# forgi86/pyMPC

Measured on AMD Instinct MI355X. Metric: QP-solves/sec (MPC steps/sec) at nx=12 nu=4 Np=30; max |u*-u*_ref|, higher is better.
Workload: dtype f64

## Files before the change

### pympc_amd/csrc/mpcqp_latw.h

```cpp
#pragma once

constexpr int latw_owner(int , int , int kind, int t) { return kind == 1 ? NWAVES - 1 - t % NWAVES : t % NWAVES; }
constexpr bool latw_fused(int N) { return (N + 3) / 4 == NWAVES; }
constexpr int LATW_F0 = 6;
constexpr int LATW_FB = 6;
constexpr int latw_slot(int N, int W, int Lq, int kq, int tq) {
    int s = latw_fused(N) ? LATW_F0 : 0;
    for (int pass = 0; pass < 2; ++pass)
        for (int li = 0; li < 2; ++li) {
            const int L = pass == 0 ? li : 1 - li;
            for (int kind = (pass == 0 ? 0 : 2); kind < (pass == 0 ? 2 : 3); ++kind)
                for (int t = 0; t < lat_count(N, L, kind); ++t) {
                    if (latw_fused(N) && L == 0 && kind < 2) continue;
                    if (latw_fused(N) && kind == 2) continue;
                    if (L == Lq && kind == kq && t == tq) return s;
                    if (latw_owner(N, L, kind, t) == W) s += lat_nfr(N, L, kind, t);
                }
        }
    return s;
}
constexpr int latw_back_base(int N, int W) { return latw_slot(N, W, -1, -1, -1); }
constexpr int latw_slots(int N, int W) { return latw_slot(N, W, -1, -1, -1) + (latw_fused(N) ? LATW_FB : 0); }
constexpr int latw_max_slots(int N) { int m = 0; for (int w = 0; w < NWAVES; ++w) m = latw_slots(N, w) > m ? latw_slots(N, w) : m; return m; }
constexpr int latw_top_stage(int r) { return 4 * (r + 1) - 1; }

#define LATW_TOP_LDS(N) ((BcrFmt::top_count(N) * BcrFmt::top_count(N) + 2) * BcrFmt::NN + 32 * BcrFmt::top_count(N))
#if NT == 512
#define LATW_DISPATCH(wv, CALL) switch (wv) { \
    case 0: { constexpr int W = 0; CALL; } break; case 1: { constexpr int W = 1; CALL; } break; \
    case 2: { constexpr int W = 2; CALL; } break; case 3: { constexpr int W = 3; CALL; } break; \
    case 4: { constexpr int W = 4; CALL; } break; case 5: { constexpr int W = 5; CALL; } break; \
    case 6: { constexpr int W = 6; CALL; } break; default: { constexpr int W = 7; CALL; } break; }
#else
#define LATW_DISPATCH(wv, CALL) LAT_DISPATCH(wv, CALL)
#endif

template <int N, int W>
__device__ __forceinline__ void latw_load(const double *F, d4 *fr) {
    const int lane = threadIdx.x & 63;
    if constexpr (latw_fused(N)) {
        constexpr int s0 = 4 * W;
        if constexpr (s0 < N) { fr[0] = bcr_frag(F, s0, BcrFmt::ODINV, lane); fr[2] = bcr_frag(F, s0, BcrFmt::OLBRT, lane); }
        if constexpr (s0 + 2 < N) { fr[1] = bcr_frag(F, s0 + 2, BcrFmt::ODINV, lane); fr[3] = bcr_frag(F, s0 + 2, BcrFmt::OLBLT, lane); }
        if constexpr (s0 + 3 < N) fr[4] = bcr_frag(F, s0 + 2, BcrFmt::OLBRT, lane);
        if constexpr (W > 0 && s0 < N) fr[5] = bcr_frag(F, s0, BcrFmt::OLBLT, lane);
    }
    if constexpr (latw_fused(N)) {
        constexpr int bb = latw_back_base(N, W), e1 = 4 * W + 1, ea = 4 * W, eb = 4 * W + 2;
        if constexpr (e1 < N) { if constexpr (e1 - 2 >= 0) fr[bb] = bcr_frag(F, e1, BcrFmt::OLBL, lane); if constexpr (e1 + 2 < N) fr[bb + 1] = bcr_frag(F, e1, BcrFmt::OLBR, lane); }
        if constexpr (ea < N) { if constexpr (ea - 1 >= 0) fr[bb + 2] = bcr_frag(F, ea, BcrFmt::OLBL, lane); if constexpr (ea + 1 < N) fr[bb + 3] = bcr_frag(F, ea, BcrFmt::OLBR, lane); }
        if constexpr (eb < N) { fr[bb + 4] = bcr_frag(F, eb, BcrFmt::OLBL, lane); if constexpr (eb + 1 < N) fr[bb + 5] = bcr_frag(F, eb, BcrFmt::OLBR, lane); }
    }
    static_for<0, 2>([&](auto lc) {
        constexpr int L = decltype(lc)::value, h = 1 << L;
        static_for<0, lat_count(N, L, 0)>([&](auto tc) {
            constexpr int t = decltype(tc)::value, i = lat_stage(L, 0, t);
            if constexpr (!(latw_fused(N) && L == 0) && latw_owner(N, L, 0, t) == W) {
                constexpr int s = latw_slot(N, W, L, 0, t);
                fr[s] = bcr_frag(F, i - h, BcrFmt::OLBRT, lane);
                if constexpr (i + h < N) fr[s + 1] = bcr_frag(F, i + h, BcrFmt::OLBLT, lane);
            }
        });
        static_for<0, lat_count(N, L, 1)>([&](auto tc) {
            constexpr int t = decltype(tc)::value, e = lat_stage(L, 1, t);
            if constexpr (!(latw_fused(N) && L == 0) && latw_owner(N, L, 1, t) == W) { constexpr int s1 = latw_slot(N, W, L, 1, t); fr[s1] = bcr_frag(F, e, BcrFmt::ODINV, lane); }
            if constexpr (!latw_fused(N) && latw_owner(N, L, 2, t) == W) {
                constexpr int s = latw_slot(N, W, L, 2, t);
                if constexpr (e - h >= 0) fr[s] = bcr_frag(F, e, BcrFmt::OLBL, lane);
                constexpr int s2 = s + (e - h >= 0 ? 1 : 0);
                if constexpr (e + h < N) fr[s2] = bcr_frag(F, e, BcrFmt::OLBR, lane);
            }
        });
    });
}

struct LatwVecs { double *tb, *cb; const double *t1, *t2, *t3, *c1, *c2, *c3; double *xt, *x2; };
template <bool FROMC>
__device__ __forceinline__ void latw_mv_lds(const d4 a, const LatwVecs &v, int off, double &p, double &q) {
    const double i0 = FROMC ? v.cb[off] : v.tb[off], i1 = FROMC ? v.c1[off] : v.t1[off], i2 = FROMC ? v.c2[off] : v.t2[off], i3 = FROMC ? v.c3[off] : v.t3[off];
    p = __builtin_amdgcn_mfma_f64_4x4x4f64(a[0], i0, p, 0, 0, 0);
    q = __builtin_amdgcn_mfma_f64_4x4x4f64(a[2], i2, q, 0, 0, 0);
    p = __builtin_amdgcn_mfma_f64_4x4x4f64(a[1], i1, p, 0, 0, 0);
    q = __builtin_amdgcn_mfma_f64_4x4x4f64(a[3], i3, q, 0, 0, 0);
}

template <int N, int W, int L>
__device__ __forceinline__ void latw_fwd(const d4 *fr, const LatwVecs &v) {
    constexpr int h = 1 << L;
    static_for<0, lat_count(N, L, 0)>([&](auto tc) {
        constexpr int t = decltype(tc)::value, i = lat_stage(L, 0, t);
        if constexpr (latw_owner(N, L, 0, t) == W) {
            constexpr int s = latw_slot(N, W, L, 0, t);
            double p = v.tb[i * 16], q = 0.0;
            if constexpr (latw_fused(N) && L == 1) p += v.x2[((i + 1) / 4 - 1) * 16];
            latw_mv_lds<false>(fr[s], v, (i - h) * 16, p, q);
            if constexpr (i + h < N) latw_mv_lds<false>(fr[s + 1], v, (i + h) * 16, p, q);
            if constexpr (L == 1) v.xt[((i + 1) / 4 - 1) * 16] = p + q;
            else v.tb[i * 16] = p + q;
        }
    });
    static_for<0, lat_count(N, L, 1)>([&](auto tc) {
        constexpr int t = decltype(tc)::value, e = lat_stage(L, 1, t);
        if constexpr (latw_owner(N, L, 1, t) == W) {
            constexpr int s1 = latw_slot(N, W, L, 1, t);
            double p = 0.0, q = 0.0;
            latw_mv_lds<false>(fr[s1], v, e * 16, p, q);
            v.cb[e * 16] = p + q;
        }
    });
}
template <int N, int W>
__device__ __forceinline__ void latw_fwd0_own(const d4 *fr, const LatwVecs &v) {
    constexpr int s0 = 4 * W;
    if constexpr (s0 < N) { double p = 0.0, q = 0.0; latw_mv_lds<false>(fr[0], v, s0 * 16, p, q); v.cb[s0 * 16] = p + q; }
    if constexpr (s0 + 2 < N) { double p = 0.0, q = 0.0; latw_mv_lds<false>(fr[1], v, (s0 + 2) * 16, p, q); v.cb[(s0 + 2) * 16] = p + q; }
    if constexpr (s0 + 1 < N) {
        double p = v.tb[(s0 + 1) * 16], q = 0.0;
        latw_mv_lds<false>(fr[2], v, s0 * 16, p, q);
        if constexpr (s0 + 2 < N) latw_mv_lds<false>(fr[3], v, (s0 + 2) * 16, p, q);
        v.tb[(s0 + 1) * 16] = p + q;
    }
    if constexpr (s0 + 3 < N) { double p = v.tb[(s0 + 3) * 16], q = 0.0; latw_mv_lds<false>(fr[4], v, (s0 + 2) * 16, p, q); v.tb[(s0 + 3) * 16] = p + q; }
    if constexpr (W > 0 && s0 < N) { double p = 0.0, q = 0.0; latw_mv_lds<false>(fr[5], v, s0 * 16, p, q); v.x2[(W - 1) * 16] = p + q; }
}
template <int N, int W, int L, bool TOPIN>
__device__ __forceinline__ void latw_bwd(const d4 *fr, const LatwVecs &v) {
    constexpr int h = 1 << L;
    static_for<0, lat_count(N, L, 2)>([&](auto tc) {
        constexpr int t = decltype(tc)::value, e = lat_stage(L, 2, t);
        if constexpr (latw_owner(N, L, 2, t) == W) {
            constexpr int s = latw_slot(N, W, L, 2, t), s2 = s + (e - h >= 0 ? 1 : 0);
            double p = v.cb[e * 16], q = 0.0;
            if constexpr (e - h >= 0) latw_mv_lds<TOPIN>(fr[s], v, (e - h) * 16, p, q);
            if constexpr (e + h < N) latw_mv_lds<TOPIN>(fr[s2], v, (e + h) * 16, p, q);
            v.tb[e * 16] = p + q;
        }
    });
}

template <int N, int W>
__device__ __forceinline__ void latw_bwd1(const d4 *fr, const LatwVecs &v) {
    static_for<0, BcrFmt::top_count(N)>([&](auto rc) {
        constexpr int r = decltype(rc)::value;
        if constexpr (r % NWAVES == W) v.tb[latw_top_stage(r) * 16] = v.cb[latw_top_stage(r) * 16];
    });
    latw_bwd<N, W, 1, true>(fr, v);
}

template <int N, int W>
__device__ __forceinline__ void latw_bwd_own(const d4 *fr, const LatwVecs &v) {
    constexpr int bb = latw_back_base(N, W), e1 = 4 * W + 1, ea = 4 * W, eb = 4 * W + 2;
    if constexpr (W < BcrFmt::top_count(N)) v.tb[latw_top_stage(W) * 16] = v.cb[latw_top_stage(W) * 16];
    if constexpr (e1 < N) {
        double p = v.cb[e1 * 16], q = 0.0;
        if constexpr (e1 - 2 >= 0) latw_mv_lds<true>(fr[bb], v, (e1 - 2) * 16, p, q);
        if constexpr (e1 + 2 < N) latw_mv_lds<true>(fr[bb + 1], v, (e1 + 2) * 16, p, q);
        v.tb[e1 * 16] = p + q;
    }
    if constexpr (ea < N) {
        double p = v.cb[ea * 16], q = 0.0;
        if constexpr (ea - 1 >= 0) latw_mv_lds<true>(fr[bb + 2], v, (ea - 1) * 16, p, q);
        if constexpr (ea + 1 < N) latw_mv_lds<false>(fr[bb + 3], v, (ea + 1) * 16, p, q);
        v.tb[ea * 16] = p + q;
    }
    if constexpr (eb < N) {
        double p = v.cb[eb * 16], q = 0.0;
        latw_mv_lds<false>(fr[bb + 4], v, (eb - 1) * 16, p, q);
        if constexpr (eb + 1 < N) latw_mv_lds<true>(fr[bb + 5], v, (eb + 1) * 16, p, q);
        v.tb[eb * 16] = p + q;
    }
}

typedef double d2 __attribute__((ext_vector_type(2)));
__device__ __forceinline__ d4 latw_top_frag(const double *TopL, int blk, int lane) {
    const d2 lo = *(const d2 *)(TopL + ((blk * 2 + 0) * 64 + lane) * 2), hi = *(const d2 *)(TopL + ((blk * 2 + 1) * 64 + lane) * 2);
    return d4{lo[0], lo[1], hi[0], hi[1]};
}

template <int CTRL>
__device__ __forceinline__ double latw_dpp(double x) {
    const long long xi = __builtin_bit_cast(long long, x);
    const int lo = DPP_MOVE((int)xi, CTRL), hi = DPP_MOVE((int)(xi >> 32), CTRL);
    return __builtin_bit_cast(double, ((long long)hi << 32) | (unsigned)lo);
}
template <int N, int W>
__device__ __forceinline__ void latw_top_valu(const double *TopL, const double *Xt, double *Cc, int lane) {
    constexpr int NTOP = BcrFmt::top_count(N), H = 2;
    static_for<0, NTOP>([&](auto rc) {
        constexpr int r = decltype(rc)::value;
        if constexpr (r % NWAVES == W) {
            const d2 *tm = (const d2 *)TopL + (size_t)(r * 2 * NTOP) * 64 + lane;
            constexpr int KQ = NTOP, NA = NTOP < 4 ? NTOP : 4, NG = (KQ + H - 1) / H;
            const d2 *xv = (const d2 *)(Xt + 2 * NTOP * (lane & 7));
            double a0[NA], a1[NA];
            d2 bx[2][H], b0[2][H], b1[2][H];
            auto load = [&](auto gc) {
                constexpr int g = decltype(gc)::value, k0 = g * H, n = (k0 + H < KQ ? k0 + H : KQ) - k0;
                static_for<0, n>([&](auto jc) { constexpr int j = decltype(jc)::value, k = k0 + j; bx[g & 1][j] = xv[k]; b0[g & 1][j] = tm[k * 64]; b1[g & 1][j] = tm[(NTOP + k) * 64]; });
            };
            auto compute = [&](auto gc) {
                constexpr int g = decltype(gc)::value, k0 = g * H, n = (k0 + H < KQ ? k0 + H : KQ) - k0;
                static_for<0, n>([&](auto jc) {
                    constexpr int j = decltype(jc)::value, k = k0 + j, q = k % NA;
                    const d2 x = bx[g & 1][j], t0 = b0[g & 1][j], t1 = b1[g & 1][j];
                    if constexpr (k < NA) { a0[q] = t0[0] * x[0]; a1[q] = t1[0] * x[0]; }
                    else { a0[q] = fma(t0[0], x[0], a0[q]); a1[q] = fma(t1[0], x[0], a1[q]); }
                    a0[q] = fma(t0[1], x[1], a0[q]); a1[q] = fma(t1[1], x[1], a1[q]);
                });
            };
            __builtin_amdgcn_sched_barrier(0);
            load(std::integral_constant<int, 0>{});
            __builtin_amdgcn_sched_barrier(0);
            static_for<0, NG>([&](auto gc) {
                constexpr int g = decltype(gc)::value;
                if constexpr (g + 1 < NG) load(std::integral_constant<int, g + 1>{});
                __builtin_amdgcn_sched_barrier(0);
                compute(gc);
                __builtin_amdgcn_sched_barrier(0);
            });
            double s0 = a0[0], s1 = a1[0];
            if constexpr (NA == 4) { s0 = (a0[0] + a0[1]) + (a0[2] + a0[3]); s1 = (a1[0] + a1[1]) + (a1[2] + a1[3]); }
            else { static_for<1, NA>([&](auto jc) { constexpr int j = decltype(jc)::value; s0 += a0[j]; s1 += a1[j]; }); }
            s0 += latw_dpp<0xB1>(s0); s1 += latw_dpp<0xB1>(s1);
            s0 += latw_dpp<0x4E>(s0); s1 += latw_dpp<0x4E>(s1);
            s0 += latw_dpp<0x141>(s0); s1 += latw_dpp<0x141>(s1);
            if ((lane & 7) == 0) *(d2 *)(Cc + latw_top_stage(r) * 16 + 2 * (lane >> 3)) = d2{s0, s1};
        }
    });
}

template <int N>
__device__ __forceinline__ void latw_solve(const d4 *fr, const double *TopL, const LatwVecs &v, double *Cc, int wv, int lane) {
    constexpr int NTOP = BcrFmt::top_count(N);
    static_assert(bcr_levels(N) >= 3 && NTOP >= 1, "two levels of reduction, then the dense top");
    if constexpr (!latw_fused(N)) {
        LATW_DISPATCH(wv, (latw_fwd<N, W, 0>(fr, v)))
        __syncthreads();
    }
    TICK(1)
    LATW_DISPATCH(wv, (latw_fwd<N, W, 1>(fr, v)))
    __syncthreads();
    TICK(2)
    LATW_DISPATCH(wv, (latw_top_valu<N, W>(TopL, TopL + LATW_TOP_LDS(N) - 32 * NTOP, Cc, lane)))
    __syncthreads();
    TICK(3)
    if constexpr (latw_fused(N)) {
        LATW_DISPATCH(wv, (latw_bwd_own<N, W>(fr, v)))
        TICK(4)
    } else {
        LATW_DISPATCH(wv, (latw_bwd1<N, W>(fr, v)))
        __syncthreads();
        TICK(4)
        LATW_DISPATCH(wv, (latw_bwd<N, W, 0, false>(fr, v)))
    }
}

enum { LATW_CONTINUE = 0, LATW_SOLVED = 1, LATW_GENERIC = 2 };
template <int NXT, int NUT, int NST>
__device__ int latw_check(double pv, double pv2, double ncq, double zA, double ysA, double omA, double zB, double ysB, double omB, double z0, double ys0, double om0,
                          double loA, double hiA, double loB, double hiB, double cc, int iter, int *frame_pin);
template <int NXT, int NUT, int NST>
__device__ int latw_carry(int iter, int *frame_pin);

template <int NXT, int NUT, int NST>
__device__ __forceinline__ int admm_latw(const Lay &L, const HotPtrs &P, Smem &S, double *Xl, double *Zl, double *Yl, double alpha, int iters, int iter0) {
    constexpr int NB = 16, N = NST, NG = (N + 3) / 4, QN = (NG + NWAVES - 1) / NWAVES;
#ifdef MPCQP_RUN_TIMING
    const unsigned long long tf0_ = clock64();
#endif
    const bool fast = iter0 >= 0 && L.hot_lds > L.hot_sz;
    static_assert(NXT + NUT <= NB, "16 x 16 stages");
    const int nx = NXT ? NXT : L.nx, nu = NUT ? NUT : L.nu, NR = L.N;
    const int b = inst_of(P.perm), tid = threadIdx.x, lane = tid & 63, wv = __builtin_amdgcn_readfirstlane(tid >> 6);
    gdouble *gx = (gdouble *)(P.x + (size_t)b * L.n), *gz = (gdouble *)(P.z + (size_t)b * L.m), *gy = (gdouble *)(P.y + (size_t)b * L.m);
    cgdouble *om = (cgdouble *)(P.omega + (size_t)b * L.m), *sv = (cgdouble *)(P.s + (size_t)b * L.n), *qv = (cgdouble *)S.Qv;
    gdouble *dxg = (gdouble *)(P.dx + (size_t)b * L.n), *dyg = (gdouble *)(P.dy + (size_t)b * L.m);
    const double cc = P.c[b], cinv = 1.0 / cc, beta = 1.0 - alpha;
    const double *hot = S.hot;
    constexpr int VS = LAT_VS(N);
    double *Tc = S.T + NB, *Cc = Tc + VS, *WA = Cc + VS, *WB = WA + VS;
    double *TopL = Yl + L.m + ((smem_common_doubles(L) + L.n + 2 * L.m) & 1);
    TICK_RESET
    TICK_START
#ifdef MPCQP_RUN_TIMING
    if (tid == 0) atomicAdd(&g_ticks[12], clock64() - tf0_);
#endif
    for (int i = tid; i < LAT_LDS_DOUBLES(N); i += NT) S.T[i] = 0.0;
    const double *Fb = P.F + (size_t)b * P.fsz;
    constexpr int NTOP = BcrFmt::top_count(N);
    if (S.iflag[2] == 0) {
        typedef __attribute__((address_space(1))) const d2 cgd2;
        cgd2 *Fv = (cgd2 *)(Fb + BcrFmt::topv_off(N));
        {
            constexpr int PAIRS = NTOP * NTOP * 128, TRIPS = (PAIRS + NT - 1) / NT;
            d2 buf[TRIPS];
#pragma unroll
            for (int t = 0; t < TRIPS; ++t) { const int idx = tid + t * NT; buf[t] = Fv[idx < PAIRS ? idx : PAIRS - 1]; }
#pragma unroll
            for (int t = 0; t < TRIPS; ++t) { const int idx = tid + t * NT; if (idx < PAIRS) *(d2 *)(TopL + 2 * idx) = buf[t]; }
        }
        const double *Ad = hot + L.oAd, *Bd = hot + L.oBd;
        auto gent = [&](int r, int c) { return r < nx ? (c < nx ? Ad[r * nx + c] : (c < nx + nu ? Bd[r * nu + (c - nx)] : 0.0)) : 0.0; };
        if (wv == 0) {
            const d4 g = lat_make_frag(lane, gent);
            *(d2 *)(TopL + (((NTOP * NTOP) * 2 + 0) * 64 + lane) * 2) = d2{g[0], g[1]}; *(d2 *)(TopL + (((NTOP * NTOP) * 2 + 1) * 64 + lane) * 2) = d2{g[2], g[3]};
        } else if (wv == 1) {
            const d4 g = lat_make_frag(lane, [&](int r, int c) { return gent(c, r); });
            *(d2 *)(TopL + (((NTOP * NTOP + 1) * 2 + 0) * 64 + lane) * 2) = d2{g[0], g[1]}; *(d2 *)(TopL + (((NTOP * NTOP + 1) * 2 + 1) * 64 + lane) * 2) = d2{g[2], g[3]};
        }
        __syncthreads();
        if (tid == 0) S.iflag[2] = 1;
    }
    d4 fr[latw_max_slots(N)];
    const int lo16 = vec_lane_offset(lane);
    const int lI = lane >> 4, lB = (lane >> 2) & 3;
    const int o1 = 4 * ((lB + 1) & 3) + lI, o2 = 4 * ((lB + 2) & 3) + lI, o3 = 4 * ((lB + 3) & 3) + lI;
    const LatwVecs vec{Tc + lo16, Cc + lo16, Tc + o1, Tc + o2, Tc + o3, Cc + o1, Cc + o2, Cc + o3, TopL + LATW_TOP_LDS(N) - 32 * BcrFmt::top_count(N) + lo16, TopL + LATW_TOP_LDS(N) - 16 * BcrFmt::top_count(N) + lo16};
    const int a = 4 * ((lane >> 2) & 3) + (lane >> 4), J = lane & 3;
    const bool is_x = a < nx;
    const int jj = a - nx;
    const double cef = cc * hot[L.oeps];
    double pv[QN], pv2[QN], svp[QN], ncq[QN], sve[QN], kap[QN], okap[QN], te[QN], loA[QN], hiA[QN], loB[QN], hiB[QN];
    LatRow rA[QN], rB[QN], r0{0.0, 0.0, 0.0, 1.0};
    int sl[QN], pidx[QN], aidx[QN], bidx[QN];
    bool ok[QN];
#pragma unroll
    for (int q = 0; q < QN; ++q) {
        const int g = wv + NWAVES * q, s = g < NG ? 4 * g + J : 4 * NG;
        sl[q] = s * NB + a;
        ok[q] = is_x ? s < NR : (a < nx + nu && s < NR - 1);
        const int e = s * nx + a, cu = s * nu + jj;
        pidx[q] = is_x ? e : L.ou + cu; aidx[q] = is_x ? e : L.ri + cu; bidx[q] = is_x ? L.rs + e : L.rdu + nu + cu;
        te[q] = 0.0;
        const bool live = ok[q], sx = live && is_x && L.soft;
        const int ip = live ? pidx[q] : 0, ia = live ? aidx[q] : 0, ib = live ? bidx[q] : 0, iq = live ? (is_x ? e : L.n_x + cu) : 0, ie = sx ? L.oe + e : 0;
        const double g_pv = gx[ip], g_sv = sv[ip], g_q = qv[iq], g_oA = om[ia], g_zA = gz[ia], g_yA = gy[ia], g_oB = om[ib], g_zB = gz[ib], g_yB = gy[ib];
        const double g_pe = gx[ie], g_se = sv[ie];
        const int jc = (jj >= 0 && jj < nu) ? jj : 0, ac = a < nx ? a : 0;
        const double b_x0 = S.x0s[ac], b_xlo = hot[L.oxmin + ac], b_xhi = hot[L.oxmax + ac];
        const double b_ulo = hot[L.oumin + jc], b_uhi = hot[L.oumax + jc], b_dlo = hot[L.oDumin + jc], b_dhi = hot[L.oDumax + jc];
        pv[q] = live ? g_pv : 0.0; svp[q] = live ? g_sv : 0.0; ncq[q] = live ? -cc * g_q : 0.0;
        rA[q] = LatRow{0.0, 0.0, 0.0, 1.0}; rB[q] = LatRow{0.0, 0.0, 0.0, 1.0};
        if (live) {
            rA[q].om = g_oA; rA[q].z = g_zA; rA[q].ys = cc * g_yA / g_oA; rA[q].w = g_oA * (g_zA - rA[q].ys);
            rB[q].om = g_oB; rB[q].z = g_zB; rB[q].ys = cc * g_yB / g_oB; rB[q].w = g_oB * (g_zB - rB[q].ys);
        }
        pv2[q] = sx ? g_pe : 0.0; sve[q] = sx ? g_se : 0.0;
        kap[q] = sx ? 1.0 / (cef + g_se + g_oB) : 0.0; okap[q] = sx ? g_oB * kap[q] : 0.0;
        loA[q] = live ? (is_x ? (s == 0 ? -b_x0 : 0.0) : b_ulo) : 0.0; hiA[q] = live ? (is_x ? (s == 0 ? -b_x0 : 0.0) : b_uhi) : 0.0;
        loB[q] = live ? (is_x ? b_xlo : b_dlo) : 0.0; hiB[q] = live ? (is_x ? b_xhi : b_dhi) : 0.0;
    }
    const bool u0v = wv == 0 && J == 0 && !is_x && a < nx + nu;
    {
        const int i0 = L.rdu + ((jj >= 0 && jj < nu) ? jj : 0);
        const double o0 = om[i0], z0 = gz[i0], y0 = gy[i0];
        if (u0v) { r0.om = o0; r0.z = z0; r0.ys = cc * y0 / o0; r0.w = o0 * (z0 - r0.ys); }
    }
    const int onext = (jj + 1 < nu) ? 1 : NB - nu + 1, oprev = (jj > 0) ? -1 : -(NB - nu + 1);
    const double selx = is_x ? 1.0 : 0.0, sgnA = is_x ? -1.0 : 1.0;
    __syncthreads();
#pragma unroll
    for (int q = 0; q < QN; ++q) { WA[sl[q]] = rA[q].w; WB[sl[q]] = rB[q].w; }
    __syncthreads();
    TICK(8)
    int iter = iter0 >= 0 ? iter0 : 0, term = 0;
    for (;;) {
    TICK_START
    { const double *Fr = opaque_ptr(Fb); LATW_DISPATCH(wv, (latw_load<N, W>(Fr, fr))) }
    TICK(7)
    for (int it = 1; it <= iters; ++it) {
        const bool keep_delta = it == iters;
        TICK_START
        {
            double g[QN], h2[QN];
#pragma unroll
            for (int q = 0; q < QN; ++q) { g[q] = 0.0; h2[q] = 0.0; lat_mv(latw_top_frag(TopL, NTOP * NTOP + 1, lane), WA[sl[q] + NB], g[q], h2[q]); }
#pragma unroll
            for (int q = 0; q < QN; ++q) {
                const double wprev = WB[sl[q] + oprev];
                te[q] = fma(sve[q], pv2[q], rB[q].w) * kap[q];
                const double viaB = is_x ? fma(-rB[q].om, te[q], rB[q].w) : wprev - rB[q].w;
                double rhs = fma(svp[q], pv[q], ncq[q]) + (g[q] + h2[q]);
                rhs = fma(sgnA, rA[q].w, rhs) + viaB;
                if (q == 0) rhs += r0.w;
                Tc[sl[q]] = ok[q] ? rhs : 0.0;
            }
        }
        if constexpr (latw_fused(N)) { LATW_DISPATCH(wv, (latw_fwd0_own<N, W>(fr, vec))) }
        __syncthreads();
        TICK(0)
        latw_solve<N>(fr, TopL, vec, Cc, wv, lane);
        __syncthreads();
        TICK(5)
        {
            double g[QN], h2[QN];
#pragma unroll
            for (int q = 0; q < QN; ++q) { g[q] = 0.0; h2[q] = 0.0; lat_mv(latw_top_frag(TopL, NTOP * NTOP, lane), Tc[sl[q] - NB], g[q], h2[q]); }
#pragma unroll
            for (int q = 0; q < QN; ++q) {
                const double xt = Tc[sl[q]], un = Tc[sl[q] + onext];
                const double et = fma(-okap[q], xt, te[q]);
                const double vn = fma(alpha, xt, beta * pv[q]), en = fma(alpha, et, beta * pv2[q]);
                const double ztA = fma(selx, (g[q] + h2[q]) - xt - xt, xt);
                const double ztB = is_x ? xt + et : un - xt;
                const double dA = lat_row_step(rA[q], ztA, loA[q], hiA[q], alpha, beta);
                const double dB = lat_row_step(rB[q], ztB, loB[q], hiB[q], alpha, beta);
                if (keep_delta && ok[q]) {
                    const int ip = opaque_lane(pidx[q]), ia = opaque_lane(aidx[q]), ib = opaque_lane(bidx[q]);
                    dxg[ip] = vn - pv[q];
                    if (is_x && L.soft) dxg[ip + L.oe] = en - pv2[q];
                    dyg[ia] = (rA[q].om * cinv) * dA; dyg[ib] = (rB[q].om * cinv) * dB;
                }
                pv[q] = vn; pv2[q] = en;
                if (q == 0 && u0v) { const double d0 = lat_row_step(r0, xt, S.du0[jj], S.du0[nu + jj], alpha, beta); if (keep_delta) dyg[opaque_lane(L.rdu + jj)] = (r0.om * cinv) * d0; }
                WA[sl[q]] = ok[q] ? rA[q].w : 0.0; WB[sl[q]] = ok[q] ? rB[q].w : 0.0;
            }
        }
        __syncthreads();
        TICK(6)
    }
    iter += iters;
    if (!fast) break;
    TICK_START
    if constexpr (QN != 1) break;
    else {
        const RunArgs &R = run_kargs().R;
        if (stop_mode(iter, R.max_iter, R.chk, R.rho_every, R.plain != 0) != COLD_CHECK) break;
        int verdict;
        { FramePin pin; verdict = latw_check<NXT, NUT, NST>(pv[0], pv2[0], ncq[0], rA[0].z, rA[0].ys, rA[0].om, rB[0].z, rB[0].ys, rB[0].om, r0.z, r0.ys, r0.om,
                                                               loA[0], hiA[0], loB[0], hiB[0], cc, iter, &pin.v); }
        verdict = __builtin_amdgcn_readfirstlane(verdict);
        if (verdict == LATW_SOLVED) {
            const int kc = __builtin_amdgcn_readfirstlane(S.iflag[6]), ke = __builtin_amdgcn_readfirstlane(S.iflag[7]);
            if (!(R.nsteps > 0 && kc >= 0 && ke <= R.nsteps && kc + 1 < ke)) { term = 1; break; }
            int carried;
            { FramePin pin; carried = latw_carry<NXT, NUT, NST>(iter, &pin.v); }
            if (!__builtin_amdgcn_readfirstlane(carried)) { term = 1; break; }
            if (u0v) ncq[0] = Tc[sl[0]];
            if (is_x && wv == 0 && (lane & 3) == 0) { loA[0] = Cc[sl[0]]; hiA[0] = loA[0]; }
            iter = 0;
        } else if (verdict != LATW_CONTINUE) break;
        iters = next_stop(iter, R.max_iter, R.chk, R.rho_every) - iter;
        auto rt = [&](LatRow &r) { r.ys = cc * (r.ys * (r.om * cinv)) / r.om; r.w = r.om * (r.z - r.ys); };
        rt(rA[0]); rt(rB[0]);
        if (u0v) rt(r0);
        WA[sl[0]] = ok[0] ? rA[0].w : 0.0; WB[sl[0]] = ok[0] ? rB[0].w : 0.0;
        __syncthreads();
    }
    TICK(9)
    }
    TICK_START
    if (!term) {
        auto put_row = [&](const LatRow &r, int idx) { const double y = r.ys * (r.om * cinv); gz[idx] = r.z; gy[idx] = y; Zl[idx] = r.z; Yl[idx] = y; };
#pragma unroll
        for (int q = 0; q < QN; ++q) {
            if (ok[q]) {
                gx[pidx[q]] = pv[q]; Xl[pidx[q]] = pv[q];
                if (is_x && L.soft) { gx[pidx[q] + L.oe] = pv2[q]; Xl[pidx[q] + L.oe] = pv2[q]; }
                put_row(rA[q], aidx[q]); put_row(rB[q], bidx[q]);
            }
        }
        if (u0v) put_row(r0, L.rdu + jj);
    }
    if (tid == 0) S.iflag[5] = iter;
    TICK(9)
    TICK_FLUSH
#ifdef MPCQP_RUN_TIMING
    if (tid == 0) atomicAdd(&g_ticks[11], clock64() - tf0_);
#endif
    return term;
}
```

Before: 2.115 million.

## Reuse the computed e1 result in the fused backward pass and add deferral options

In the fused backward-own step, the freshly computed stage-e1 vector is kept in registers. Its four block reads are reloaded once, or rotated in-register when LATW_HANDOFF is set, and reused by both neighbour products instead of each rereading LDS. New LATW_DEFER options let the level-0/1 column products run inside the dense top VALU stage so their MFMAs overlap its loads. Both macros default to 0, so by default only the register reuse of the e1 reads is active, which removes one set of LDS reads.

```diff
diff --git a/pympc_amd/csrc/mpcqp_latw.h b/pympc_amd/csrc/mpcqp_latw.h
--- a/pympc_amd/csrc/mpcqp_latw.h
+++ b/pympc_amd/csrc/mpcqp_latw.h
@@ -1,4 +1,10 @@
 #pragma once
+#ifndef LATW_DEFER
+#define LATW_DEFER 0
+#endif
+#ifndef LATW_HANDOFF
+#define LATW_HANDOFF 0
+#endif
 
 constexpr int latw_owner(int , int , int kind, int t) { return kind == 1 ? NWAVES - 1 - t % NWAVES : t % NWAVES; }
 constexpr bool latw_fused(int N) { return (N + 3) / 4 == NWAVES; }
@@ -75,13 +81,32 @@
 }
 
 struct LatwVecs { double *tb, *cb; const double *t1, *t2, *t3, *c1, *c2, *c3; double *xt, *x2; };
+struct LatwIn { double i0, i1, i2, i3; };
+__device__ __forceinline__ void latw_mv_in(const d4 a, const LatwIn &x, double &p, double &q) {
+    p = __builtin_amdgcn_mfma_f64_4x4x4f64(a[0], x.i0, p, 0, 0, 0);
+    q = __builtin_amdgcn_mfma_f64_4x4x4f64(a[2], x.i2, q, 0, 0, 0);
+    p = __builtin_amdgcn_mfma_f64_4x4x4f64(a[1], x.i1, p, 0, 0, 0);
+    q = __builtin_amdgcn_mfma_f64_4x4x4f64(a[3], x.i3, q, 0, 0, 0);
+}
 template <bool FROMC>
-__device__ __forceinline__ void latw_mv_lds(const d4 a, const LatwVecs &v, int off, double &p, double &q) {
-    const double i0 = FROMC ? v.cb[off] : v.tb[off], i1 = FROMC ? v.c1[off] : v.t1[off], i2 = FROMC ? v.c2[off] : v.t2[off], i3 = FROMC ? v.c3[off] : v.t3[off];
-    p = __builtin_amdgcn_mfma_f64_4x4x4f64(a[0], i0, p, 0, 0, 0);
-    q = __builtin_amdgcn_mfma_f64_4x4x4f64(a[2], i2, q, 0, 0, 0);
-    p = __builtin_amdgcn_mfma_f64_4x4x4f64(a[1], i1, p, 0, 0, 0);
-    q = __builtin_amdgcn_mfma_f64_4x4x4f64(a[3], i3, q, 0, 0, 0);
+__device__ __forceinline__ LatwIn latw_in(const LatwVecs &v, int off) {
+    return LatwIn{FROMC ? v.cb[off] : v.tb[off], FROMC ? v.c1[off] : v.t1[off], FROMC ? v.c2[off] : v.t2[off], FROMC ? v.c3[off] : v.t3[off]};
+}
+template <bool FROMC>
+__device__ __forceinline__ void latw_mv_lds(const d4 a, const LatwVecs &v, int off, double &p, double &q) { latw_mv_in(a, latw_in<FROMC>(v, off), p, q); }
+
+constexpr int latw_def_task(int N, int W) { for (int t = 0; t < lat_count(N, 1, 1); ++t) if (latw_owner(N, 1, 1, t) == W) return t; return -1; }
+constexpr int latw_def_stage(int N, int W, int k) {
+    if (k < 2) return 4 * W + 2 * k < N ? 4 * W + 2 * k : -1;
+    return latw_def_task(N, W) < 0 ? -1 : lat_stage(1, 1, latw_def_task(N, W));
+}
+constexpr int latw_def_slot(int N, int W, int k) { return k < 2 ? k : latw_slot(N, W, 1, 1, latw_def_task(N, W)); }
+template <int N, int W, int K0, int K1>
+__device__ __forceinline__ void latw_def_now(const d4 *fr, const LatwVecs &v) {
+    static_for<K0, K1>([&](auto kc) {
+        constexpr int k = decltype(kc)::value, e = latw_def_stage(N, W, k);
+        if constexpr (e >= 0) { double p = 0.0, q = 0.0; latw_mv_lds<false>(fr[latw_def_slot(N, W, k)], v, e * 16, p, q); v.cb[e * 16] = p + q; }
+    });
 }
 
 template <int N, int W, int L>
@@ -101,7 +126,7 @@
     });
     static_for<0, lat_count(N, L, 1)>([&](auto tc) {
         constexpr int t = decltype(tc)::value, e = lat_stage(L, 1, t);
-        if constexpr (latw_owner(N, L, 1, t) == W) {
+        if constexpr (latw_owner(N, L, 1, t) == W && !(LATW_DEFER && latw_fused(N) && L == 1)) {
             constexpr int s1 = latw_slot(N, W, L, 1, t);
             double p = 0.0, q = 0.0;
             latw_mv_lds<false>(fr[s1], v, e * 16, p, q);
@@ -112,8 +137,7 @@
 template <int N, int W>
 __device__ __forceinline__ void latw_fwd0_own(const d4 *fr, const LatwVecs &v) {
     constexpr int s0 = 4 * W;
-    if constexpr (s0 < N) { double p = 0.0, q = 0.0; latw_mv_lds<false>(fr[0], v, s0 * 16, p, q); v.cb[s0 * 16] = p + q; }
-    if constexpr (s0 + 2 < N) { double p = 0.0, q = 0.0; latw_mv_lds<false>(fr[1], v, (s0 + 2) * 16, p, q); v.cb[(s0 + 2) * 16] = p + q; }
+    if constexpr (!LATW_DEFER) latw_def_now<N, W, 0, 2>(fr, v);
     if constexpr (s0 + 1 < N) {
         double p = v.tb[(s0 + 1) * 16], q = 0.0;
         latw_mv_lds<false>(fr[2], v, s0 * 16, p, q);
@@ -151,21 +175,28 @@
 __device__ __forceinline__ void latw_bwd_own(const d4 *fr, const LatwVecs &v) {
     constexpr int bb = latw_back_base(N, W), e1 = 4 * W + 1, ea = 4 * W, eb = 4 * W + 2;
     if constexpr (W < BcrFmt::top_count(N)) v.tb[latw_top_stage(W) * 16] = v.cb[latw_top_stage(W) * 16];
+    LatwIn x1{0.0, 0.0, 0.0, 0.0};
     if constexpr (e1 < N) {
         double p = v.cb[e1 * 16], q = 0.0;
         if constexpr (e1 - 2 >= 0) latw_mv_lds<true>(fr[bb], v, (e1 - 2) * 16, p, q);
         if constexpr (e1 + 2 < N) latw_mv_lds<true>(fr[bb + 1], v, (e1 + 2) * 16, p, q);
-        v.tb[e1 * 16] = p + q;
+        x1.i0 = p + q;
+        v.tb[e1 * 16] = x1.i0;
+#if LATW_HANDOFF
+        x1.i1 = rot_blocks<1>(x1.i0); x1.i2 = rot_blocks<2>(x1.i0); x1.i3 = rot_blocks<3>(x1.i0);
+#else
+        x1 = latw_in<false>(v, e1 * 16);
+#endif
     }
     if constexpr (ea < N) {
         double p = v.cb[ea * 16], q = 0.0;
         if constexpr (ea - 1 >= 0) latw_mv_lds<true>(fr[bb + 2], v, (ea - 1) * 16, p, q);
-        if constexpr (ea + 1 < N) latw_mv_lds<false>(fr[bb + 3], v, (ea + 1) * 16, p, q);
+        if constexpr (ea + 1 < N) latw_mv_in(fr[bb + 3], x1, p, q);
         v.tb[ea * 16] = p + q;
     }
     if constexpr (eb < N) {
         double p = v.cb[eb * 16], q = 0.0;
-        latw_mv_lds<false>(fr[bb + 4], v, (eb - 1) * 16, p, q);
+        latw_mv_in(fr[bb + 4], x1, p, q);
         if constexpr (eb + 1 < N) latw_mv_lds<true>(fr[bb + 5], v, (eb + 1) * 16, p, q);
         v.tb[eb * 16] = p + q;
     }
@@ -183,9 +214,10 @@
     const int lo = DPP_MOVE((int)xi, CTRL), hi = DPP_MOVE((int)(xi >> 32), CTRL);
     return __builtin_bit_cast(double, ((long long)hi << 32) | (unsigned)lo);
 }
-template <int N, int W>
-__device__ __forceinline__ void latw_top_valu(const double *TopL, const double *Xt, double *Cc, int lane) {
+template <int N, int W, int K0, int K1>
+__device__ __forceinline__ void latw_top_valu(const double *TopL, const double *Xt, double *Cc, int lane, const d4 *fr, const LatwVecs &v) {
     constexpr int NTOP = BcrFmt::top_count(N), H = 2;
+    if constexpr (K0 < K1 && W % NWAVES >= NTOP) latw_def_now<N, W, K0, K1>(fr, v);
     static_for<0, NTOP>([&](auto rc) {
         constexpr int r = decltype(rc)::value;
         if constexpr (r % NWAVES == W) {
@@ -208,12 +240,20 @@
                     a0[q] = fma(t0[1], x[1], a0[q]); a1[q] = fma(t1[1], x[1], a1[q]);
                 });
             };
+            static_assert(K1 - K0 <= NG && (K0 == K1 || NTOP <= NWAVES), "one deferred product per group of the row");
+            LatwIn din[3]; double dp[3] = {0.0, 0.0, 0.0}, dq[3] = {0.0, 0.0, 0.0};
+            auto dread = [&](auto kc) { constexpr int k = decltype(kc)::value; if constexpr (k >= K0 && k < K1) if constexpr (latw_def_stage(N, W, k) >= 0) din[k] = latw_in<false>(v, latw_def_stage(N, W, k) * 16); };
+            auto dmul = [&](auto kc) { constexpr int k = decltype(kc)::value; if constexpr (k >= K0 && k < K1) if constexpr (latw_def_stage(N, W, k) >= 0) latw_mv_in(fr[latw_def_slot(N, W, k)], din[k], dp[k], dq[k]); };
+            auto dstore = [&](auto kc) { constexpr int k = decltype(kc)::value; if constexpr (latw_def_stage(N, W, k) >= 0) v.cb[latw_def_stage(N, W, k) * 16] = dp[k] + dq[k]; };
             __builtin_amdgcn_sched_barrier(0);
+            static_for<K0, K1>(dread);
             load(std::integral_constant<int, 0>{});
             __builtin_amdgcn_sched_barrier(0);
+            if constexpr (K0 < K1) { static_for<K0, K1>(dmul); __builtin_amdgcn_sched_barrier(0); }
             static_for<0, NG>([&](auto gc) {
                 constexpr int g = decltype(gc)::value;
                 if constexpr (g + 1 < NG) load(std::integral_constant<int, g + 1>{});
+                if constexpr (g == 0) static_for<K0, K1>(dstore);
                 __builtin_amdgcn_sched_barrier(0);
                 compute(gc);
                 __builtin_amdgcn_sched_barrier(0);
@@ -238,10 +278,12 @@
         __syncthreads();
     }
     TICK(1)
-    LATW_DISPATCH(wv, (latw_fwd<N, W, 1>(fr, v)))
+    constexpr bool DEF = LATW_DEFER && latw_fused(N);
+    constexpr int TK0 = !DEF ? 0 : LATW_DEFER == 2 ? 2 : 0, TK1 = DEF ? 3 : 0;
+    LATW_DISPATCH(wv, (latw_fwd<N, W, 1>(fr, v), latw_def_now<N, W, 0, (DEF && LATW_DEFER == 2 ? 2 : 0)>(fr, v)))
     __syncthreads();
     TICK(2)
-    LATW_DISPATCH(wv, (latw_top_valu<N, W>(TopL, TopL + LATW_TOP_LDS(N) - 32 * NTOP, Cc, lane)))
+    LATW_DISPATCH(wv, (latw_top_valu<N, W, TK0, TK1>(TopL, TopL + LATW_TOP_LDS(N) - 32 * NTOP, Cc, lane, fr, v)))
     __syncthreads();
     TICK(3)
     if constexpr (latw_fused(N)) {
```

Result: no change. 2.123 million (median of 2 runs) (+0.4%).
